# izhengfan/se2lam

Measured on AMD Instinct MI355X. Metric: BA GN-iters/s (200 KF, 20k pts), higher is better.
Workload: dtype f64; 1 GPU; globalBA-window 200 KF / 20000 landmarks / 119817 EdgeSE2XYZ + 199 PreEdgeSE2, LM optimize(10) (config 4 formulation, SURVEY D3); parallelism=single GPU

## Files before the change

### include/se2gpu.h

```cpp
#ifndef SE2GPU_H
#define SE2GPU_H

#include <stddef.h>
#include <stdint.h>

#ifdef __cplusplus
extern "C" {
#endif

#define SE2GPU_OK 0
#define SE2GPU_ERR_INVALID (-1)
#define SE2GPU_ERR_NO_DEVICE (-2)
#define SE2GPU_ERR_HIP (-3)
#define SE2GPU_ERR_CAPACITY (-4)
#define SE2GPU_ERR_STATE (-5)

const char* se2gpu_last_error(void);
int se2gpu_device_count(void);
const char* se2gpu_version(void);

typedef struct se2gpu_orb se2gpu_orb;

typedef struct se2gpu_orb_params {
    int32_t nfeatures;
// ... 255 lines not shown
#define SE2GPU_BA_GN 1
int se2gpu_ba_optimize(se2gpu_ba* h, int iters, int mode, const volatile uint8_t* stop_flag, int verbose,
                       se2gpu_ba_stats* stats);
int se2gpu_ba_optimize_batch(se2gpu_ba** handles, int count, int iters, int mode, const volatile uint8_t* stop_flag,
                             se2gpu_ba_stats* stats);
int se2gpu_ba_last_batch_path(void);
int se2gpu_ba_get_se2(se2gpu_ba* h, int id, double xyt[3]);
int se2gpu_ba_get_xyz(se2gpu_ba* h, int id, double xyz[3]);
int se2gpu_ba_get_all(se2gpu_ba* h, double* poses , double* lms );
double se2gpu_ba_chi2(se2gpu_ba* h);

int se2gpu_ba_debug_reduced_system(se2gpu_ba* h, double lambda, double* S, double* bs);
int se2gpu_ba_debug_solve(se2gpu_ba* h, double lambda, double* x, int* factor_ok);
int se2gpu_ba_debug_solver_path(const se2gpu_ba* h);
int se2gpu_ba_debug_linearize_counts(const se2gpu_ba* h, int* runs, int* skips, long long* twin_bytes);
int se2gpu_ba_debug_pool_sizes(int out2[2]);
int se2gpu_ba_debug_chol_verify(se2gpu_ba* h, unsigned long long* counts2, unsigned long long* records, int cap);
int se2gpu_ba_debug_solve_plan(int P, int D, const uint8_t* pattern, int allow_nd, int* nsys, int* nbc, int* depth, int* ntask,
                               int* ndep, int32_t* pose_off, int32_t* tasks4, int task_cap, int32_t* deps, int dep_cap);
int se2gpu_ba_debug_solve_plan_tile(int P, int D, const uint8_t* pattern, int allow_nd, int tile, int* nsys, int* nbc, int* depth, int* ntask,
                                    int* ndep, int32_t* pose_off, int32_t* tasks4, int task_cap, int32_t* deps, int dep_cap);
int se2gpu_ba_debug_solve_plan_neager(int P, int D, const uint8_t* pattern, int allow_nd, int tile, int32_t* neager, int cap);
int se2gpu_ba_debug_plan_neager(se2gpu_ba* h, int* nsys, int* permuted, int* ntask, int32_t* neager, int cap);

int se2gpu_triangulate(int n, const se2gpu_keypoint* kps_ref, const se2gpu_keypoint* kps_cur, int n_cur,
                       int32_t* match_idx, const uint8_t* has_observation, const float* P_ref, const float* P_cur,
                       const float* Ocam, float lower_depth, float upper_depth, int min_degree, float* pos_out,
                       uint8_t* good_parallax, int* n_good, int* n_tracked_old);

typedef struct se2gpu_track se2gpu_track;
int se2gpu_track_create(se2gpu_track** out);
void se2gpu_track_destroy(se2gpu_track* h);
int se2gpu_track_fundamental_mask(se2gpu_track* h, const float* pt1, const float* pt2, int n, uint8_t* mask,
                                  int* n_inliers);
int se2gpu_track_remove_outliers(se2gpu_track* h, const se2gpu_keypoint* kps1, int n1, const se2gpu_keypoint* kps2,
                                 int n2, int32_t* matches, int* n_inliers);
int se2gpu_track_last_ransac(const se2gpu_track* h, int info[4]);
int se2gpu_track_set_stream(se2gpu_track* h, void* hip_stream);
void* se2gpu_track_stream(se2gpu_track* h);
int se2gpu_track_sync(se2gpu_track* h);

int se2gpu_track_loop_verify_batch_device(se2gpu_track* h,
                                          const se2gpu_keypoint* d_kps, const int32_t* d_counts, int cap, int nframes,
                                          const uint8_t* d_has_mp ,
                                          const int32_t* d_num_mps ,
                                          const int32_t* d_pair_a, const int32_t* d_pair_b, int npairs,
// ... 123 lines not shown
```

### se2lam_amd/capi.py

```python
from __future__ import annotations

import ctypes as C
import os

import numpy as np

HERE = os.path.dirname(os.path.abspath(__file__))
LIB_PATH = os.path.join(HERE, "lib", "libse2gpu.so")

OK = 0
ERR_INVALID, ERR_NO_DEVICE, ERR_HIP, ERR_CAPACITY, ERR_STATE = -1, -2, -3, -4, -5


class Se2GpuError(RuntimeError):
    def __init__(self, code, msg):
        super().__init__(f"se2gpu error {code}: {msg}")
        self.code = code


class Keypoint(C.Structure):
    _fields_ = [("x", C.c_float), ("y", C.c_float), ("size", C.c_float), ("angle", C.c_float),
                ("response", C.c_float), ("octave", C.c_int32), ("class_id", C.c_int32)]


# ... 151 lines not shown
    "se2gpu_feat_edge_batch": (_I, [_I, _I, _I, _I, _VP, _VP, _D, _D, _D, _VP, _VP, _VP, _VP, _D, _D, _VP, _VP, _VP, _VP, _VP,
                                    _VP, _VP, _VP]),
    "se2gpu_ba_initialize": (_I, [_VP]),
    "se2gpu_ba_set_edge_level": (_I, [_VP, _I, _I]),
    "se2gpu_ba_reset_estimates": (_I, [_VP]),
    "se2gpu_ba_reset_estimates_batch": (_I, [_VP, _I]),
    "se2gpu_ba_optimize": (_I, [_VP, _I, _I, _PU8, _I, C.POINTER(BaStats)]),
    "se2gpu_ba_optimize_batch": (_I, [C.POINTER(_VP), _I, _I, _I, _PU8, C.POINTER(BaStats)]),
    "se2gpu_ba_last_batch_path": (_I, []),
    "se2gpu_ba_get_se2": (_I, [_VP, _I, _PD]),
    "se2gpu_ba_get_xyz": (_I, [_VP, _I, _PD]),
    "se2gpu_ba_get_all": (_I, [_VP, _PD, _PD]),
    "se2gpu_ba_chi2": (_D, [_VP]),
    "se2gpu_ba_debug_reduced_system": (_I, [_VP, _D, _PD, _PD]),
    "se2gpu_ba_debug_solve": (_I, [_VP, _D, _PD, C.POINTER(C.c_int)]),
    "se2gpu_ba_debug_solver_path": (_I, [_VP]),
    "se2gpu_ba_debug_linearize_counts": (_I, [_VP, C.POINTER(C.c_int), C.POINTER(C.c_int), C.POINTER(C.c_longlong)]),
    "se2gpu_ba_debug_chol_verify": (_I, [_VP, _VP, _VP, _I]),
    "se2gpu_ba_debug_pool_sizes": (_I, [_VP]),
    "se2gpu_ba_debug_solve_plan": (_I, [_I, _I, _VP, _I, _VP, _VP, _VP, _VP, _VP, _VP, _VP, _I, _VP, _I]),
    "se2gpu_ba_debug_solve_plan_tile": (_I, [_I, _I, _VP, _I, _I, _VP, _VP, _VP, _VP, _VP, _VP, _VP, _I, _VP, _I]),
    "se2gpu_ba_debug_solve_plan_neager": (_I, [_I, _I, _VP, _I, _I, _VP, _I]),
    "se2gpu_ba_debug_plan_neager": (_I, [_VP, C.POINTER(C.c_int), C.POINTER(C.c_int), C.POINTER(C.c_int), _VP, _I]),
    "se2gpu_triangulate": (_I, [_I, _VP, _VP, _I, _VP, _VP, _VP, _VP, _VP, C.c_float, C.c_float, _I, _VP, _VP,
                           C.POINTER(C.c_int), C.POINTER(C.c_int)]),
    "se2gpu_track_create": (_I, [C.POINTER(_VP)]),
    "se2gpu_track_destroy": (None, [_VP]),
    "se2gpu_track_fundamental_mask": (_I, [_VP, _VP, _VP, _I, _VP, C.POINTER(C.c_int)]),
    "se2gpu_track_remove_outliers": (_I, [_VP, _VP, _I, _VP, _I, _VP, C.POINTER(C.c_int)]),
    "se2gpu_track_last_ransac": (_I, [_VP, _VP]),
    "se2gpu_track_set_stream": (_I, [_VP, _VP]),
    "se2gpu_track_stream": (_VP, [_VP]),
    "se2gpu_track_sync": (_I, [_VP]),
    "se2gpu_track_loop_verify_batch_device": (_I, [_VP, _VP, _VP, _I, _I, _VP, _VP, _VP, _VP, _I, _VP, _VP, _VP, _VP]),
    "se2gpu_plane_motion_prior": (_I, [_VP, _VP, _D, _D, _D, _VP, _VP]),
    "se2gpu_track_pose_ba": (_I, [_VP, _VP, _VP, _VP, _I, _VP, _VP, _VP, _D, _D, _D, _D, _I, _VP, C.POINTER(BaStats)]),
    "se2gpu_track_triangulate": (_I, [_VP, _I, _VP, _VP, _I, _VP, _VP, _VP, _VP, _VP, C.c_float, C.c_float, _I, _VP, _VP,
                                 C.POINTER(C.c_int), C.POINTER(C.c_int)]),
    "se2gpu_ba_reduce_buffer_doubles": (_SZ, [_VP, _I]),
    "se2gpu_ba_exchange_doubles": (_SZ, [_I]),
    "se2gpu_ba_exchange_doubles_h": (_SZ, [_VP]),
    "se2gpu_ba_exchange_row": (_I, [_I, C.POINTER(C.c_size_t), C.POINTER(C.c_int)]),
    "se2gpu_ba_set_allreduce": (_I, [_VP, ALLREDUCE_FN, _VP, _VP]),
    "se2gpu_ba_set_shard": (_I, [_VP, _I, _I]),
    "se2gpu_comm_unique_id": (_I, [_VP]),
    "se2gpu_comm_create": (_I, [_VP, _I, _I, C.POINTER(_VP)]),
# ... 208 lines not shown
```

### se2lam_amd/csrc/ba.hip

```cpp
#include <algorithm>
#include <atomic>
#include <chrono>
#include <cmath>
#include <cstdlib>
#include <functional>
#include <limits>
#include <mutex>
#include <thread>
#include <memory>
#include <unordered_map>

#include "common.h"
#include "se3_math.h"
#include "ba_device.h"
#include "ba3_device.h"
#include "ba_window.h"

using namespace se2gpu;
using namespace se2gpu::badev;

namespace {



// ... 591 lines not shown
    }
}

constexpr int kGrpPerWG = 28;
constexpr int kChunk = 16;

struct Reduce2Args {
    int P, ld, nwg_off;
    double lambda;
    int root;
    const int4* grp;
    const int *blk_a, *blk_b, *pair_i, *pair_j, *blk_odo;
    const double *W, *Dg;
    const uint8_t* fixed;
    const int *pose_ptr, *pose_edges, *podo_ptr, *podo_item, *o_i, *o_j;
    const double *o_meas, *o_info, *poses;
    double *S, *bp;
    const BaCtl* ctl;
    const double* poses_b;
    unsigned* epoch;
    const int* pose_off;
    int nsys;
    const double *W_alt, *Dg_alt;
};
__device__ __forceinline__ void d_reduce2(const unsigned bx, const Reduce2Args& ra) {
    const double *W = ra.W, *Dg = ra.Dg, *poses = ra.poses;
    if (ra.ctl && ra.ctl->rec_sel) { W = ra.W_alt; Dg = ra.Dg_alt; }
    double lambda = ra.lambda;
    const int n = ra.pose_off ? ra.nsys : 3 * ra.P;
    __shared__ double part[kGrpPerWG][9];
    __shared__ double dpart[kBlock / 64][12];
    const int ndiag = (ra.P + 1 + 7) & ~7;
    if ((int)bx >= ndiag) {
        const int bid = (int)bx - ndiag;
        const int nwg_pad = (ra.nwg_off + 7) & ~7;
        const int wg = (bid & 7) * (nwg_pad >> 3) + (bid >> 3);
        if (wg >= ra.nwg_off) return;
        const int lane = threadIdx.x & 63, gw = lane / 9, en = lane - 9 * gw;
        const int g = gw < 7 ? (int)(threadIdx.x >> 6) * 7 + gw : kGrpPerWG;
        int4 d = make_int4(-1, 0, 0, 0);
        if (g < kGrpPerWG) d = ra.grp[(size_t)wg * kGrpPerWG + g];
        if (ra.ctl) {
            if (ra.ctl->done) return;
            if (ra.ctl->sel) poses = ra.poses_b;
        }
        const int r = en / 3, c = en - 3 * r;
        double acc0 = 0, acc1 = 0;
        int a = 0, b = 0, od = -1, ca = 0, cb = 0;
        bool free_ab = false;
        if (d.x >= 0) {
            const int gb = 9 * gw, t8 = min(en, 7);
            int q0 = min(d.y + t8, d.z - 1), q1 = min(d.y + 8 + t8, d.z - 1);
            int my_i0 = 0, my_j0 = 0, my_i1 = 0, my_j1 = 0;
            if (d.z > d.y) { my_i0 = ra.pair_i[q0]; my_j0 = ra.pair_j[q0]; my_i1 = ra.pair_i[q1]; my_j1 = ra.pair_j[q1]; }
            a = ra.blk_a[d.x];
            b = ra.blk_b[d.x];
            od = ra.blk_odo[d.x];
            free_ab = !ra.fixed[a] && !ra.fixed[b];
            ca = ra.pose_off ? ra.pose_off[a] : 3 * a;
            cb = ra.pose_off ? ra.pose_off[b] : 3 * b;
            for (int q = d.y; q < d.z; q += 8) {
                const bool second = ((q - d.y) & 8) != 0;
                if (!second && q != d.y) {
                    q0 = min(q + t8, d.z - 1); q1 = min(q + 8 + t8, d.z - 1);
                    my_i0 = ra.pair_i[q0]; my_j0 = ra.pair_j[q0]; my_i1 = ra.pair_i[q1]; my_j1 = ra.pair_j[q1];
                }
                const int my_i = second ? my_i1 : my_i0, my_j = second ? my_j1 : my_j0;
                double wi[8], wj[8];
#pragma unroll
                for (int u = 0; u < 8; ++u) {
                    const int ia = __shfl(my_i, gb + u), ib = __shfl(my_j, gb + u);
                    wi[u] = W[(size_t)ia * 9 + en];
                    wj[u] = W[(size_t)ib * 9 + en];
                }
#pragma unroll
                for (int u = 0; u < 8; u += 2) {
                    const double w0 = (q + u < d.z) ? 1.0 : 0.0, w1 = (q + u + 1 < d.z) ? 1.0 : 0.0;
                    double y[2][3], hh[2][3];
#pragma unroll
                    for (int k = 0; k < 3; ++k) {
                        y[0][k] = __shfl(wi[u], gb + 3 * r + k);
                        hh[0][k] = __shfl(wj[u], gb + 3 * c + k);
                        y[1][k] = __shfl(wi[u + 1], gb + 3 * r + k);
                        hh[1][k] = __shfl(wj[u + 1], gb + 3 * c + k);
                    }
                    acc0 += w0 * (y[0][0] * hh[0][0] + y[0][1] * hh[0][1] + y[0][2] * hh[0][2]);
                    acc1 += w1 * (y[1][0] * hh[1][0] + y[1][1] * hh[1][1] + y[1][2] * hh[1][2]);
                }
            }
            part[g][en] = acc0 + acc1;
        }
        __syncthreads();
        if (d.x >= 0 && (d.w & 0xff) == g) {
            const int ng = d.w >> 8;
            double tot = 0;
            for (int t = 0; t < ng; ++t) tot += part[g + t][en];
            double out = 0.0;
            if (free_ab) {
                out = -tot;
                if (od >= 0) {
                    double e[3], A[9], B[9], WA[9], WB[9], omr[3];
                    odo_terms(poses, ra.fixed, ra.o_i, ra.o_j, ra.o_meas, ra.o_info, od >> 1, e, A, B, WA, WB, omr);
                    const int rr = (od & 1) ? c : r, cc = (od & 1) ? r : c;
                    const double a0 = rr == 0 ? A[0] : (rr == 1 ? A[1] : A[2]), a1 = rr == 0 ? A[3] : (rr == 1 ? A[4] : A[5]),
                                 a2 = rr == 0 ? A[6] : (rr == 1 ? A[7] : A[8]);
                    const double b0 = cc == 0 ? WB[0] : (cc == 1 ? WB[1] : WB[2]), b1 = cc == 0 ? WB[3] : (cc == 1 ? WB[4] : WB[5]),
                                 b2 = cc == 0 ? WB[6] : (cc == 1 ? WB[7] : WB[8]);
                    out += a0 * b0 + a1 * b1 + a2 * b2;
                }
            }
            ra.S[(size_t)(ca + r) * ra.ld + cb + c] = out;
            ra.S[(size_t)(cb + c) * ra.ld + ca + r] = out;
        }
        return;
    }
    if (ra.ctl) {
        if (ra.ctl->done) return;
        if (ra.ctl->sel) poses = ra.poses_b;
        lambda = ra.ctl->lambda;
    }
    const int p = (int)bx;
    if (p > ra.P) return;
    const int lane = threadIdx.x & 63, wv = threadIdx.x >> 6;
    double* __restrict__ bs = ra.S + (size_t)n * ra.ld;
    if (p == ra.P) {
        for (size_t t = (size_t)n * ra.ld + n + threadIdx.x; t < (size_t)ra.ld * ra.ld; t += kBlock) ra.S[t] = 0.0;
        if (threadIdx.x == 0) {
            ra.S[(size_t)ra.ld * ra.ld + 2] = 0.0;
            *ra.epoch += 1u;
        }
        return;
// ... 66 lines not shown
            for (int q = 0; q < 3; ++q) {
                const double j0 = isj ? B[3 * q] : A[3 * q], j1 = isj ? B[3 * q + 1] : A[3 * q + 1], j2 = isj ? B[3 * q + 2] : A[3 * q + 2];
                const double w0 = isj ? WB[3 * q] : WA[3 * q], w1 = isj ? WB[3 * q + 1] : WA[3 * q + 1], w2 = isj ? WB[3 * q + 2] : WA[3 * q + 2];
                jr[q] = r == 0 ? j0 : (r == 1 ? j1 : j2);
                wc[q] = i < 9 ? (c == 0 ? w0 : (c == 1 ? w1 : w2)) : omr[q];
            }
            v += jr[0] * wc[0] + jr[1] * wc[1] + jr[2] * wc[2];
        }
        if (i < 9) {
            const int r = i / 3, c = i - 3 * r;
            double out;
            if (fa) out = (r == c && ra.root) ? 1.0 : 0.0;
            else out = v + ((r == c && ra.root) ? lambda : 0.0);
            const int cp = ra.pose_off ? ra.pose_off[p] : 3 * p;
            ra.S[(size_t)(cp + r) * ra.ld + cp + c] = out;
        } else {
            const int r = i - 9;
            const double gz = dpart[0][9 + r] + dpart[1][9 + r] + dpart[2][9 + r] + dpart[3][9 + r];
            bs[(ra.pose_off ? ra.pose_off[p] : 3 * p) + r] = fa ? 0.0 : v - gz;
            ra.bp[(size_t)p * 3 + r] = fa ? 0.0 : v;
        }
    }
}
__global__ __launch_bounds__(kBlock) void k_reduce2(Reduce2Args a) {
    d_reduce2(blockIdx.x, a);
}

__global__ void k_reduce_odo(int O, int ld, const int* __restrict__ o_i, const int* __restrict__ o_j,
                             const double* __restrict__ Oij, double* __restrict__ S, const int* __restrict__ pose_off) {
    const int t = blockIdx.x * blockDim.x + threadIdx.x;
    if (t >= O * 9) return;
    const int k = t / 9, r = (t % 9) / 3, c = t % 3;
    const int i = o_i[k], j = o_j[k];
    const double v = Oij[t];
    if (v == 0.0) return;
    const int ci = pose_off ? pose_off[i] : 3 * i, cj = pose_off ? pose_off[j] : 3 * j;
    atomicAdd(&S[(size_t)(ci + r) * ld + cj + c], v);
    atomicAdd(&S[(size_t)(cj + c) * ld + ci + r], v);
}

constexpr int kNB = 32;
constexpr int kSlabs = 4;
constexpr int kSlabDoubles = 2 * kNB * 8;
__host__ __device__ inline size_t pub_tile(int kind, int i, int j, int nt, int nbc) {
    return ((size_t)(kind * nt + i) * nbc + j) * (kSlabs * kSlabDoubles);
}
inline size_t chol_work_doubles(int ld) {
// ... 1847 lines not shown
    int bulk_E = 0;
    const int32_t *bulk_kf = nullptr, *bulk_lm = nullptr;
    const double *bulk_uv = nullptr, *bulk_info = nullptr;
    bool lg_active = false;
    std::vector<float> lg_lc, lg_lw, lg_sigma2, lg_Rcw, lg_twb;
    float lg_fx = 0, lg_srot = 0, lg_sz = 0;
    DevBuf<float> d_lg_lc, d_lg_lw, d_lg_sigma2, d_lg_Rcw, d_lg_twb;
    std::vector<EdgeOdo> odo;
    bool initialized = false;
    unsigned long init_serial = 0;
    hipEvent_t join_event = nullptr;
    hipStream_t join_stream = nullptr;
    bool own_pending = false;
    int P = 0, L = 0, E = 0, O = 0, nblk = 0, nparts = 0;
    int ld = 0;
    bool host_solve = false;
    DevBuf<double> poses0, lms0, poses_a, poses_b, lms_a, lms_b;
    double *poses = nullptr, *poses_t = nullptr, *lms = nullptr, *lms_t = nullptr;
    DevBuf<uint8_t> fixed;
    DevBuf<int> lm_ptr, e_kf, e_lm, pose_ptr, pose_edges, podo_ptr, podo_item, o_i, o_j;
    DevBuf<int> blk_a, blk_b, blk_ptr, pair_i, pair_j, blk_odo;
    DevBuf<int4> grp;
    int nwg_off = 0, grp_cap_wg = 0;
    DevBuf<uint8_t> garena;
    DevBuf<int> plan_np, plan_base, plan_key0, plan_key1, plan_idx, plan_hist, plan_offs, plan_out, plan_tsum, plan_toff;
    DevBuf<int2> plan_st0, plan_st1;
    bool odo_fallback = false;
    bool odo_self_loop = false;
    DevBuf<double> e_uv, e_info, o_meas, o_info;
    DevBuf<double> Hpl, Hpp_e, bp_e, Hll, bl, Dinv, z, Y, Dg, Hpp, bp, Oii, Ojj, Oij, obi, obj;
    DevBuf<double> red_own, xp, part, scal, diag3, Rinv;
    DevBuf<double> rec_twin;
    bool run_spec = false;
    DevBuf<double> red_packed;
    DevBuf<int4> chol_tasks;
    DevBuf<int> chol_deps;
    DevBuf<int> chol_neager;
    DevBuf<int> pose_off;
    DevBuf<int> col_src;
    std::vector<int> h_pose_off;
    DevBuf<uint8_t> plan_nz;
    DevBuf<double> plan_nzd;
    PinBuf<uint8_t> h_plan_nz;
    DevBuf<uint8_t> solver_arena;
    int nsys = 0;
    int solve_depth = 0;
// ... 740 lines not shown
        const int w = w_cyc;
        for (int lv = 0; lv <= 2; ++lv) ring(w, w, lv);
        auto tiles = [&](int poses) { return (D * poses + nb - 1) / nb; };
        int sw_best = w, est_best = tiles(std::max(h - w, P - h - w)) + tiles(2 * w);
        for (int sw = w + 1; sw <= w + nb && 2 * sw + 2 * min_interior <= P; ++sw) {
            const int est = tiles(std::max(h - sw, P - h - sw)) + tiles(2 * sw);
            if (est < est_best) { est_best = est; sw_best = sw; }
        }
        if (sw_best != w) ring(w, sw_best, 0);
    }
}

int ba_copy_stream(int device, hipStream_t* out) {
    static std::mutex mu;
    static hipStream_t streams[64] = {};
    std::lock_guard<std::mutex> lk(mu);
    SE2_REQUIRE(device >= 0 && device < 64, SE2GPU_ERR_INVALID, "device %d", device);
    if (!streams[device]) SE2_HIP(hipStreamCreateWithFlags(&streams[device], hipStreamNonBlocking));
    *out = streams[device];
    return SE2GPU_OK;
}

int ba_allreduce(se2gpu_ba* h, double* ptr, size_t count);

int ba_upload_graph(se2gpu_ba* h) {
    static const bool trace = env_flag("SE2GPU_BA_INIT_TRACE", false);
    const auto t_begin = std::chrono::steady_clock::now();
    auto lap = [&](const char* what) {
        if (trace)
            std::fprintf(stderr, "[ba init] %-28s %8.1f us\n", what,
                         std::chrono::duration<double, std::micro>(std::chrono::steady_clock::now() - t_begin).count());
    };
    const int P = (int)h->pose_ids.size(), L = (int)h->lm_ids.size();
    const int E = h->bulk_E ? h->bulk_E : (int)h->he_kf.size(), O_in = h->model ? (int)h->odo3.size() : (int)h->odo.size();
    const int D = h->D, ps = h->ps, gpw = h->model ? kGrpPerWG3 : kGrpPerWG;
    const int DS = D * (D + 1) / 2;
    SE2_REQUIRE(P > 0, SE2GPU_ERR_STATE, "initialize: no pose vertices");
    SE2_REQUIRE(!h->model || (h->world == 1 && !h->allreduce), SE2GPU_ERR_STATE, "the SE3 model is single-GPU");
    SE2_REQUIRE(h->have_cam, SE2GPU_ERR_STATE, "initialize: add_cam was not called");
    SE2_REQUIRE(!h->huber_mixed, SE2GPU_ERR_INVALID, "all EdgeSE2XYZ must share one Huber delta (Map.cpp:977)");
    h->P = P; h->L = L; h->E = E; h->O = O_in;
    h->cam.huber = E ? h->huber_delta : 0.0;
    h->cam3 = Cam3{h->cam.fx, h->cam.cx, h->cam.cy, h->cam.huber};
    for (int i = 0; i < 3; ++i)
        for (int j = 0; j < 3; ++j) h->cam.Rcb[i * 3 + j] = h->Rbc[j * 3 + i];
    for (int i = 0; i < 3; ++i)
// ... 478 lines not shown
        static const bool verify = env_flag("SE2GPU_BA_CHOL_VERIFY", false);
        if (verify) {
            const size_t words = kVfyChk + 2 * 2 * kSlabs * (size_t)nt2 * nbc2;
            SE2_CHECK(h->chol_vfy.reserve(words));
            SE2_HIP(hipMemsetAsync(h->chol_vfy.p, 0, words * sizeof(unsigned long long), st));
        } else {
            h->chol_vfy.release();
        }
        h->chol_steps = env_is("SE2GPU_BA_CHOL", "steps") || nt2 > 64 || h->chol_fallback;
        if (env_flag("SE2GPU_BA_CHOL_TRACE", false)) {
            SE2_CHECK(h->chol_trace.reserve(16 * (size_t)h->chol_ntask));
            SE2_HIP(hipMemsetAsync(h->chol_trace.p, 0, 16 * (size_t)h->chol_ntask * sizeof(long long), st));
        }
        lap("solve plan");
    }
    SE2_HIP(hipStreamSynchronize(st));
    if (device_plan) {
        int nwg = 0;
        std::memcpy(&nwg, h->h_scal.p, sizeof(int));
        SE2_REQUIRE(nwg <= h->grp_cap_wg, SE2GPU_ERR_CAPACITY, "device plan: %d workgroups exceed the bound %d", nwg, h->grp_cap_wg);
        h->nwg_off = std::max(nwg, 1);
    }
    lap("synchronise");
    h->bulk_E = 0;
    h->bulk_kf = h->bulk_lm = nullptr;
    h->bulk_uv = h->bulk_info = nullptr;
    h->initialized = true;
    h->est_valid = false;
    static std::atomic<unsigned long> serial{0};
    h->init_serial = ++serial;
    drain.armed = false;
    return SE2GPU_OK;
}


int ba_join(se2gpu_ba* h, hipStream_t st, hipEvent_t* ev) {
    if (h->join_event) {
        if (h->join_stream != st) SE2_HIP(hipStreamWaitEvent(st, h->join_event, 0));
        h->join_event = nullptr;
        h->join_stream = nullptr;
    }
    if (h->own_pending && h->stream != st) {
        if (!*ev) SE2_HIP(hipEventCreateWithFlags(ev, hipEventDisableTiming));
        SE2_HIP(hipEventRecord(*ev, h->stream));
        SE2_HIP(hipStreamWaitEvent(st, *ev, 0));
        h->own_pending = false;
// ... 57 lines not shown
inline double* ba_scal(se2gpu_ba* h) { return h->red + (size_t)h->ld * h->ld; }
inline dim3 upd_grid(const se2gpu_ba* h) { return grid1((size_t)h->L * kGroup, kBlock); }
inline dim3 reduce2_grid(const se2gpu_ba* h) { return dim3(((h->P + 1 + 7) & ~7) + ((h->nwg_off + 7) & ~7)); }
LinArgs lin_args(se2gpu_ba* h, const Bufs& B, double lambda, const RecSet& alt) {
    return LinArgs{h->cam, h->L, h->lm_ptr.p, h->e_kf.p, h->e_uv.p, h->e_info.p, B.pa, h->fixed.p, B.la, h->Hpl.p, h->Hpp_e.p,
                   h->bp_e.p, h->Hll.p, h->bl.p, lambda, h->Dinv.p, h->z.p, h->Dg.p, B.c, B.pb, B.lb, alt};
}
OdoArgs odo_args(se2gpu_ba* h, const double* poses, bool ctl) {
    const Bufs B = bufs(h, ctl);
    return OdoArgs{h->O, h->o_i.p, h->o_j.p, h->o_meas.p, h->o_info.p, ctl ? B.pa : poses, h->fixed.p, h->Oii.p, h->Ojj.p, h->Oij.p,
                   h->obi.p, h->obj.p, B.c, ctl ? B.pb : nullptr};
}
PoseReduceArgs pose_reduce_args(se2gpu_ba* h) {
    return PoseReduceArgs{h->P, h->pose_ptr.p, h->pose_edges.p, h->Hpp_e.p, h->bp_e.p, h->podo_ptr.p, h->podo_item.p, h->Oii.p,
                          h->Ojj.p, h->obi.p, h->obj.p, h->Hpp.p, h->bp.p};
}
MaxdiagArgs maxdiag_args(se2gpu_ba* h, int dpp, int stride9, BaCtl* ctl) {
    return MaxdiagArgs{h->L, h->Hll.p, h->P, stride9 ? h->Hpp.p : h->diag3.p, h->fixed.p, h->scal.p, dpp, stride9, ctl};
}
Reduce2Args reduce2_args(se2gpu_ba* h, const Bufs& B, double lambda, const RecSet& alt) {
    return Reduce2Args{h->P, h->ld, h->nwg_off, lambda, h->root, h->grp.p, h->blk_a.p, h->blk_b.p, h->pair_i.p, h->pair_j.p,
                       h->blk_odo.p, h->Hpl.p, h->Dg.p, h->fixed.p, h->pose_ptr.p, h->pose_edges.p, h->podo_ptr.p, h->podo_item.p,
                       h->o_i.p, h->o_j.p, h->o_meas.p, h->o_info.p, B.pa, h->red, h->bp.p, B.c, B.pb, &h->ctl.p->epoch,
                       h->pose_off.p, h->nsys, alt.W, alt.Dg};
}
CholArgs chol_args(se2gpu_ba* h, const BaCtl* ctl, int skip, unsigned long long* head, bool verify) {
    const int n = h->nsys, ld = h->ld;
    const int nt = ld / kNB, nbc = (n + kNB - 1) / kNB;
    double* YU = h->Rinv.p + 2 * (size_t)nt * nbc * kSlabs * kSlabDoubles;
    unsigned* flagA = h->chol_flags.p;
    return CholArgs{h->red, h->Rinv.p, YU, ld, n, nbc, h->chol_tasks.p + skip, h->chol_deps.p, h->chol_neager.p + skip, h->col_src.p,
                    flagA, flagA + kSlabs * (size_t)nt * nbc, &h->ctl.p->epoch, ba_scal(h) + 2, h->chol_trace.p, ctl, h->xp.p,
                    verify ? h->chol_vfy.p : nullptr, head, h->chol_ntask - skip};
}
TrialEnd trial_end(se2gpu_ba* h, const Bufs& B, int step, int decide, int notify, double seq, bool lin = false, bool post = true) {
    return TrialEnd{ba_scal(h), post ? h->d_mail : nullptr, seq, B.c ? h->ctl.p : nullptr,
                    B.c ? (const volatile int*)h->d_stop : nullptr, step, decide, notify, lin ? 1 : 0};
}
FinArgs fin_args(se2gpu_ba* h, const Bufs& B, const double* xp, const TrialEnd& te) {
    return FinArgs{1, (int)upd_grid(h).x, h->P, h->O, h->root, h->fixed.p, xp, h->bp.p, B.pa, B.pb,
                   h->o_i.p, h->o_j.p, h->o_meas.p, h->o_info.p, h->fin_counter.p, te};
}
UpdArgs upd_args(se2gpu_ba* h, const Bufs& B, double lambda, const double* xp, const FinArgs& fin, bool lin = false) {
    return UpdArgs{h->cam, h->L, lambda, h->lm_ptr.p, h->e_kf.p, h->e_uv.p, h->e_info.p, B.pa, h->fixed.p, B.la, xp, h->z.p, h->Hpl.p,
                   h->bl.p, B.lb, h->part.p, B.c, B.pb, fin, h->Dinv.p,
                   lin ? SpecArgs{{rec_own(h), rec_twin(h)}, h->Hpp_e.p, h->bp_e.p} : SpecArgs{}};
}
// ... 1228 lines not shown
                               int* ndep, int32_t* pose_off, int32_t* tasks4, int task_cap, int32_t* deps, int dep_cap) {
    SE2_REQUIRE(P > 0 && (D == 3 || D == 6) && nsys && nbc && depth && ntask && ndep, SE2GPU_ERR_INVALID, "debug_solve_plan: bad argument");
    SolvePlan sp;
    solve_plan_choose(P, D, pattern, allow_nd != 0, sp);
    *nsys = sp.nsys; *nbc = sp.nbc; *depth = sp.depth; *ntask = (int)sp.tasks.size(); *ndep = (int)sp.deps.size();
    if (pose_off) std::memcpy(pose_off, sp.pose_off.data(), (size_t)P * 4);
    if (tasks4) {
        SE2_REQUIRE(task_cap >= (int)sp.tasks.size(), SE2GPU_ERR_CAPACITY, "debug_solve_plan: %zu tasks", sp.tasks.size());
        std::memcpy(tasks4, sp.tasks.data(), sp.tasks.size() * sizeof(int4));
    }
    if (deps) {
        SE2_REQUIRE(dep_cap >= (int)sp.deps.size(), SE2GPU_ERR_CAPACITY, "debug_solve_plan: %zu dependency entries", sp.deps.size());
        std::memcpy(deps, sp.deps.data(), sp.deps.size() * 4);
    }
    return SE2GPU_OK;
}

int se2gpu_ba_debug_solve_plan_neager(int P, int D, const uint8_t* pattern, int allow_nd, int tile, int32_t* neager, int cap) {
    SE2_REQUIRE(P > 0 && (D == 3 || D == 6) && (tile == 32 || tile == 64) && neager, SE2GPU_ERR_INVALID, "debug_solve_plan_neager: bad argument");
    SolvePlan sp;
    solve_plan_choose(P, D, pattern, allow_nd != 0, sp, false, tile);
    SE2_REQUIRE(cap >= (int)sp.neager.size(), SE2GPU_ERR_CAPACITY, "debug_solve_plan_neager: %zu tasks", sp.neager.size());
    std::memcpy(neager, sp.neager.data(), sp.neager.size() * 4);
    return SE2GPU_OK;
}

int se2gpu_ba_debug_plan_neager(se2gpu_ba* h, int* nsys, int* permuted, int* ntask, int32_t* neager, int cap) {
    SE2_REQUIRE(h && h->initialized && nsys && permuted && ntask, SE2GPU_ERR_STATE, "debug_plan_neager before initialize");
    SE2_CHECK(ba_join(h));
    SE2_HIP(hipStreamSynchronize(h->stream));
    *nsys = h->nsys; *permuted = h->col_src.p ? 1 : 0; *ntask = h->chol_ntask;
    if (neager) {
        SE2_REQUIRE(cap >= h->chol_ntask && h->chol_neager.p, SE2GPU_ERR_CAPACITY, "debug_plan_neager: %d tasks", h->chol_ntask);
        SE2_HIP(hipMemcpy(neager, h->chol_neager.p, (size_t)h->chol_ntask * 4, hipMemcpyDeviceToHost));
    }
    return SE2GPU_OK;
}

int se2gpu_ba_debug_chol_verify(se2gpu_ba* h, unsigned long long* counts2, unsigned long long* records, int cap) {
    SE2_REQUIRE(h && h->initialized && h->chol_vfy.p, SE2GPU_ERR_STATE, "the handle does not verify its hand-offs (SE2GPU_BA_CHOL_VERIFY=1)");
    SE2_CHECK(ba_join(h));
    SE2_HIP(hipStreamSynchronize(h->stream));
    unsigned long long head[8];
    SE2_HIP(hipMemcpy(head, h->chol_vfy.p, sizeof(head), hipMemcpyDeviceToHost));
    counts2[0] = head[0]; counts2[1] = head[1];
    const int nrec = (int)std::min<unsigned long long>(std::min<unsigned long long>(head[0], kVfyRecords), (unsigned long long)std::max(cap, 0));
// ... 673 lines not shown
```

Measured before the change: 7346 iters/s.

## Precompute flat per-group index records for reduce2 off-diagonal blocks

At graph upload a new kernel builds, for each reduce group, a flat 11-int4 record holding block offsets, the odometry index, the fixed flag and the pair indices, so the off-diagonal reduce path replaces chains of dependent gathers with a few contiguous loads. The odometry block term is now computed before the landmark loop and stored in shared memory, so its latency overlaps the main accumulation. The kernel also gets a min-occupancy launch bound of 5. The trade-off is extra device memory and a small setup kernel, plus possible register pressure from the occupancy hint. It is enabled by default through an environment flag.

```diff
diff --git a/include/se2gpu.h b/include/se2gpu.h
--- a/include/se2gpu.h
+++ b/include/se2gpu.h
@@ -301,6 +301,10 @@
                                     int* ndep, int32_t* pose_off, int32_t* tasks4, int task_cap, int32_t* deps, int dep_cap);
 int se2gpu_ba_debug_solve_plan_neager(int P, int D, const uint8_t* pattern, int allow_nd, int tile, int32_t* neager, int cap);
 int se2gpu_ba_debug_plan_neager(se2gpu_ba* h, int* nsys, int* permuted, int* ntask, int32_t* neager, int cap);
+int se2gpu_ba_debug_flat_records_host(int nslots, const int32_t* grp4, const int32_t* blk_a, const int32_t* blk_b, const int32_t* blk_odo,
+                                      const int32_t* pair_i, const int32_t* pair_j, const uint8_t* fixed, const int32_t* pose_off,
+                                      const int32_t* o_i, const int32_t* o_j, int32_t* flat);
+int se2gpu_ba_debug_flat_records(se2gpu_ba* h, int32_t* grp4, int32_t* flat, int cap_slots, int* nslots);
 
 int se2gpu_triangulate(int n, const se2gpu_keypoint* kps_ref, const se2gpu_keypoint* kps_cur, int n_cur,
                        int32_t* match_idx, const uint8_t* has_observation, const float* P_ref, const float* P_cur,
diff --git a/profiles/ba_reduce_flat/stamp_patch.py b/profiles/ba_reduce_flat/stamp_patch.py
--- /dev/null
+++ b/profiles/ba_reduce_flat/stamp_patch.py
@@ -0,0 +1,48 @@
+import sys
+src, dst = sys.argv[1], sys.argv[2]
+s = open(src).read()
+
+def rep(old, new, count=1):
+    global s
+    assert s.count(old) >= 1, old
+    s = s.replace(old, new, count)
+
+rep("constexpr int kFlatQ = 11;",
+    """constexpr int kFlatQ = 11;
+__device__ long long g_r2_stamps[4096 * 8];
+#define R2S(i) do { if (threadIdx.x == 0 && bx < 4096) g_r2_stamps[(size_t)bx * 8 + (i)] = wall_clock64(); } while (0)
+#define R2S_T(i, T) do { if ((int)threadIdx.x == (T) && bx < 4096) g_r2_stamps[(size_t)bx * 8 + (i)] = wall_clock64(); } while (0)
+#define R2USE(v) asm volatile("" ::"v"(v))""")
+rep("        const int wg = (bid & 7) * (nwg_pad >> 3) + (bid >> 3);\n        if (wg >= ra.nwg_off) return;",
+    "        const int wg = (bid & 7) * (nwg_pad >> 3) + (bid >> 3);\n        if (wg >= ra.nwg_off) return;\n        R2S(0);")
+rep("        const int r = en / 3, c = en - 3 * r;\n        double acc0 = 0, acc1 = 0;",
+    "        R2USE(d.x); R2USE(fq.x);\n        R2S(1);\n        const int r = en / 3, c = en - 3 * r;\n        double acc0 = 0, acc1 = 0;")
+rep("            // The block's PreEdgeSE2 term (the group that combines the block adds it): with the flat record",
+    "            R2USE(my_i0); R2USE(my_j1); R2USE(ca); R2USE(cb); R2USE(od);\n            R2S(2);\n            // The block's PreEdgeSE2 term (the group that combines the block adds it): with the flat record")
+rep("            // The group loads every word ONCE", "            R2S(3);\n            // The group loads every word ONCE")
+rep("                    acc1 += w1 * (y[1][0] * hh[1][0] + y[1][1] * hh[1][1] + y[1][2] * hh[1][2]);\n                }\n            }\n            part[g][en] = acc0 + acc1;",
+    "                    acc1 += w1 * (y[1][0] * hh[1][0] + y[1][1] * hh[1][1] + y[1][2] * hh[1][2]);\n                }\n                if (q == d.y) { R2USE(acc0); R2USE(acc1); R2S(4); }\n            }\n            R2USE(acc0); R2USE(acc1);\n            R2S(5);\n            part[g][en] = acc0 + acc1;")
+rep("        __syncthreads();\n        if (d.x >= 0 && (d.w & 0xff) == g) {\n            const int ng = d.w >> 8;",
+    "        __syncthreads();\n        R2S(6);\n        if (d.x >= 0 && (d.w & 0xff) == g) {\n            const int ng = d.w >> 8;")
+rep("            ra.S[(size_t)(cb + c) * ra.ld + ca + r] = out;\n        }\n        return;",
+    "            ra.S[(size_t)(cb + c) * ra.ld + ca + r] = out;\n            R2USE(out);\n        }\n        R2S(7);\n        return;")
+rep("    double acc[12] = {0, 0, 0, 0, 0, 0, 0, 0, 0, 0, 0, 0};  // S diag (6 sym), bp (3), g (3)",
+    "    R2S(0);\n    double acc[12] = {0, 0, 0, 0, 0, 0, 0, 0, 0, 0, 0, 0};  // S diag (6 sym), bp (3), g (3)")
+rep("            o[9 + r] = J[r] * omr[0] + J[3 + r] * omr[1] + J[6 + r] * omr[2];\n        }\n    }",
+    "            o[9 + r] = J[r] * omr[0] + J[3 + r] * omr[1] + J[6 + r] * omr[2];\n        }\n        R2S_T(3, kBlock - 8);\n    }")
+rep("                ee[u] = ra.pose_edges[e0 + min(t, ne - 1)];\n            }",
+    "                ee[u] = ra.pose_edges[e0 + min(t, ne - 1)];\n            }\n            if (base == 0) { R2USE(ee[0]); R2USE(ee[3]); R2S(1); }")
+rep("#pragma unroll\n    for (int i = 0; i < 12; ++i) acc[i] = wave_sum(acc[i]);",
+    "    R2USE(acc[0]); R2USE(acc[11]);\n    R2S(2);\n#pragma unroll\n    for (int i = 0; i < 12; ++i) acc[i] = wave_sum(acc[i]);")
+rep("    __syncthreads();\n    if (threadIdx.x < 12) {  // entries 0..8",
+    "    __syncthreads();\n    R2S(6);\n    if (threadIdx.x < 12) {  // entries 0..8")
+rep("            ra.bp[(size_t)p * 3 + r] = fa ? 0.0 : v;\n        }\n    }\n}",
+    "            ra.bp[(size_t)p * 3 + r] = fa ? 0.0 : v;\n        }\n    }\n    R2S(7);\n}")
+rep("// k_plan_flat's record builder (flat_record, the function the kernel calls) on host arrays",
+    """extern "C" int se2gpu_ba_debug_reduce_stamps(long long* out, int n) {
+    SE2_HIP(hipDeviceSynchronize());
+    SE2_HIP(hipMemcpyFromSymbol(out, HIP_SYMBOL(g_r2_stamps), (size_t)n * sizeof(long long)));
+    return SE2GPU_OK;
+}
+// k_plan_flat's record builder (flat_record, the function the kernel calls) on host arrays""")
+open(dst, "w").write(s)
diff --git a/profiles/ba_reduce_flat/stamps_summary.py b/profiles/ba_reduce_flat/stamps_summary.py
--- /dev/null
+++ b/profiles/ba_reduce_flat/stamps_summary.py
@@ -0,0 +1,33 @@
+import numpy as np, sys
+for name in ("legacy","flat"):
+    z=np.load(f"{sys.argv[1]}/stamps_{name}.npz")
+    S=z["stamps"]; P=int(z["P"]); ndiag=(P+1+7)&~7
+    print("==",name,"runs",S.shape[0],"flat_slots",int(z["flat_slots"]))
+    for run in range(S.shape[0]):
+        st=S[run].astype(np.int64)
+        valid=(st[:,0]>0)&(st[:,7]>0)
+        t0=st[valid,0].min()
+        rel=(st-t0)*0.01
+        diag=np.zeros(4096,bool); diag[:P]=True; diag&=valid
+        off=np.zeros(4096,bool); off[ndiag:]=True; off&=valid
+        end=rel[valid,7].max()
+        print(f"run {run}: valid {valid.sum()} diag {diag.sum()} off {off.sum()}  kernel span (first start -> last end) {end:.2f} us; last end: diag {rel[diag,7].max():.2f} off {rel[off,7].max():.2f}; starts: diag max {rel[diag,0].max():.2f} off max {rel[off,0].max():.2f}")
+        o=rel[off]
+        seg=[("start->record/grp",0,1),("->indices/blk",1,2),("->(odo before loop)",2,3),("->W round 1",3,4),("->all rounds",4,5),("->barrier",5,6),("->end(odo+store)",6,7)]
+        def q(x): return "med %.2f p90 %.2f max %.2f"%(np.median(x),np.percentile(x,90),x.max())
+        for nm,a,b in seg:
+            ok=(o[:,a]>-1e5)&(o[:,b]>-1e5)&(st[off][:,a]>0)&(st[off][:,b]>0)
+            print("   off %-22s %s  (n=%d)"%(nm,q(o[ok,b]-o[ok,a]),ok.sum()))
+        print("   off total                 ",q(o[:,7]-o[:,0]))
+        idx=np.argsort(o[:,7])[-max(10,len(o)//20):]
+        print("   off LAST 5%% to end: start med %.2f; tail seg (barrier->end) med %.2f max %.2f; total med %.2f"%(np.median(o[idx,0]),np.median(o[idx,7]-o[idx,6]),(o[idx,7]-o[idx,6]).max(),np.median(o[idx,7]-o[idx,0])))
+        long_tail=(o[:,7]-o[:,6])>0.8
+        print("   off wgs with barrier->end > 0.8us: %d, their end med %.2f max %.2f ; others end med %.2f max %.2f"%(long_tail.sum(), np.median(o[long_tail,7]) if long_tail.any() else -1, o[long_tail,7].max() if long_tail.any() else -1, np.median(o[~long_tail,7]), o[~long_tail,7].max()))
+        dg=rel[diag]; sd=st[diag]
+        ok1=(sd[:,1]>0)&(sd[:,2]>0)
+        print("   diag start->idx %s (n=%d)"%(q(dg[ok1,1]-dg[ok1,0]),ok1.sum()))
+        print("   diag idx->Dg gathered %s (n=%d)"%(q(dg[ok1,2]-dg[ok1,1]),ok1.sum()))
+        ok=sd[:,3]>0
+        print("   diag start->odo lanes done %s (n=%d)"%(q(dg[ok,3]-dg[ok,0]),ok.sum()))
+        print("   diag start->gather done %s"%q(dg[:,2]-dg[:,0]))
+        print("   diag gather->barrier %s ; barrier->end %s ; total %s"%(q(dg[:,6]-dg[:,2]),q(dg[:,7]-dg[:,6]),q(dg[:,7]-dg[:,0])))
diff --git a/se2lam_amd/capi.py b/se2lam_amd/capi.py
--- a/se2lam_amd/capi.py
+++ b/se2lam_amd/capi.py
@@ -197,6 +197,8 @@
     "se2gpu_ba_debug_solve_plan_tile": (_I, [_I, _I, _VP, _I, _I, _VP, _VP, _VP, _VP, _VP, _VP, _VP, _I, _VP, _I]),
     "se2gpu_ba_debug_solve_plan_neager": (_I, [_I, _I, _VP, _I, _I, _VP, _I]),
     "se2gpu_ba_debug_plan_neager": (_I, [_VP, C.POINTER(C.c_int), C.POINTER(C.c_int), C.POINTER(C.c_int), _VP, _I]),
+    "se2gpu_ba_debug_flat_records_host": (_I, [_I, _VP, _VP, _VP, _VP, _VP, _VP, _VP, _VP, _VP, _VP, _VP]),
+    "se2gpu_ba_debug_flat_records": (_I, [_VP, _VP, _VP, _I, C.POINTER(C.c_int)]),
     "se2gpu_triangulate": (_I, [_I, _VP, _VP, _I, _VP, _VP, _VP, _VP, _VP, C.c_float, C.c_float, _I, _VP, _VP,
                            C.POINTER(C.c_int), C.POINTER(C.c_int)]),
     "se2gpu_track_create": (_I, [C.POINTER(_VP)]),
diff --git a/se2lam_amd/csrc/ba.hip b/se2lam_amd/csrc/ba.hip
--- a/se2lam_amd/csrc/ba.hip
+++ b/se2lam_amd/csrc/ba.hip
@@ -637,13 +637,61 @@
     const int* pose_off;
     int nsys;
     const double *W_alt, *Dg_alt;
+    const int4* flat;
 };
+constexpr int kFlatQ = 11;
+__host__ __device__ inline void flat_record(const int4 d, const int* blk_a, const int* blk_b, const int* blk_odo,
+                                            const int* pair_i, const int* pair_j, const uint8_t* fixed, const int* pose_off,
+                                            const int* o_i, const int* o_j, int4* rec) {
+    rec[0] = d;
+    for (int t = 1; t < kFlatQ; ++t) rec[t] = make_int4(0, 0, 0, 0);
+    rec[1].z = -1;
+    if (d.x < 0) return;
+    const int a = blk_a[d.x], b = blk_b[d.x], od = blk_odo[d.x];
+    rec[1] = make_int4(pose_off ? pose_off[a] : 3 * a, pose_off ? pose_off[b] : 3 * b, od, (!fixed[a] && !fixed[b]) ? 1 : 0);
+    if (od >= 0) rec[2] = make_int4(o_i[od >> 1], o_j[od >> 1], 0, 0);
+    if (d.z > d.y)
+        for (int t = 0; t < 8; ++t) {
+            const int last = d.z - 1, q0 = d.y + t < last ? d.y + t : last, q1 = d.y + 8 + t < last ? d.y + 8 + t : last;
+            rec[3 + t] = make_int4(pair_i[q0], pair_j[q0], pair_i[q1], pair_j[q1]);
+        }
+}
+struct PlanFlatArgs {
+    int ngrp;
+    const int4* grp;
+    const int *blk_a, *blk_b, *blk_odo, *pair_i, *pair_j;
+    const uint8_t* fixed;
+    const int *pose_off, *o_i, *o_j;
+    int4* flat;
+};
+__global__ __launch_bounds__(256) void k_plan_flat(PlanFlatArgs a) {
+    const int t = blockIdx.x * 256 + threadIdx.x;
+    if (t < a.ngrp)
+        flat_record(a.grp[t], a.blk_a, a.blk_b, a.blk_odo, a.pair_i, a.pair_j, a.fixed, a.pose_off, a.o_i, a.o_j,
+                    a.flat + (size_t)t * kFlatQ);
+}
+__device__ __forceinline__ __attribute__((flatten)) void odo_terms_regs(const double pij[6], const double meas[3], const double* info, double e[3],
+                                               double A[9], double B[9], double WA[9], double WB[9], double omr[3]) {
+    const int zero = 0, one = 1;
+    odo_terms(pij, nullptr, &zero, &one, meas, info, 0, e, A, B, WA, WB, omr);
+}
+__device__ __forceinline__ double odo_block_entry(const double pij[6], const double meas[3], const double* info, int od, int r, int c) {
+    double e[3], A[9], B[9], WA[9], WB[9], omr[3];
+    odo_terms_regs(pij, meas, info, e, A, B, WA, WB, omr);
+    const int rr = (od & 1) ? c : r, cc = (od & 1) ? r : c;
+    const double a0 = rr == 0 ? A[0] : (rr == 1 ? A[1] : A[2]), a1 = rr == 0 ? A[3] : (rr == 1 ? A[4] : A[5]),
+                 a2 = rr == 0 ? A[6] : (rr == 1 ? A[7] : A[8]);
+    const double b0 = cc == 0 ? WB[0] : (cc == 1 ? WB[1] : WB[2]), b1 = cc == 0 ? WB[3] : (cc == 1 ? WB[4] : WB[5]),
+                 b2 = cc == 0 ? WB[6] : (cc == 1 ? WB[7] : WB[8]);
+    return a0 * b0 + a1 * b1 + a2 * b2;
+}
 __device__ __forceinline__ void d_reduce2(const unsigned bx, const Reduce2Args& ra) {
     const double *W = ra.W, *Dg = ra.Dg, *poses = ra.poses;
     if (ra.ctl && ra.ctl->rec_sel) { W = ra.W_alt; Dg = ra.Dg_alt; }
     double lambda = ra.lambda;
     const int n = ra.pose_off ? ra.nsys : 3 * ra.P;
     __shared__ double part[kGrpPerWG][9];
+    __shared__ double odo_part[kGrpPerWG][9];
     __shared__ double dpart[kBlock / 64][12];
     const int ndiag = (ra.P + 1 + 7) & ~7;
     if ((int)bx >= ndiag) {
@@ -653,8 +701,15 @@
         if (wg >= ra.nwg_off) return;
         const int lane = threadIdx.x & 63, gw = lane / 9, en = lane - 9 * gw;
         const int g = gw < 7 ? (int)(threadIdx.x >> 6) * 7 + gw : kGrpPerWG;
-        int4 d = make_int4(-1, 0, 0, 0);
-        if (g < kGrpPerWG) d = ra.grp[(size_t)wg * kGrpPerWG + g];
+        int4 d = make_int4(-1, 0, 0, 0), fb = make_int4(0, 0, -1, 0), fo = make_int4(0, 0, 0, 0), fq = make_int4(0, 0, 0, 0);
+        if (g < kGrpPerWG) {
+            if (ra.flat) {
+                const int4* rec = ra.flat + ((size_t)wg * kGrpPerWG + g) * kFlatQ;
+                d = rec[0]; fb = rec[1]; fo = rec[2]; fq = rec[3 + min(en, 7)];
+            } else {
+                d = ra.grp[(size_t)wg * kGrpPerWG + g];
+            }
+        }
         if (ra.ctl) {
             if (ra.ctl->done) return;
             if (ra.ctl->sel) poses = ra.poses_b;
@@ -665,15 +720,31 @@
         bool free_ab = false;
         if (d.x >= 0) {
             const int gb = 9 * gw, t8 = min(en, 7);
-            int q0 = min(d.y + t8, d.z - 1), q1 = min(d.y + 8 + t8, d.z - 1);
-            int my_i0 = 0, my_j0 = 0, my_i1 = 0, my_j1 = 0;
-            if (d.z > d.y) { my_i0 = ra.pair_i[q0]; my_j0 = ra.pair_j[q0]; my_i1 = ra.pair_i[q1]; my_j1 = ra.pair_j[q1]; }
-            a = ra.blk_a[d.x];
-            b = ra.blk_b[d.x];
-            od = ra.blk_odo[d.x];
-            free_ab = !ra.fixed[a] && !ra.fixed[b];
-            ca = ra.pose_off ? ra.pose_off[a] : 3 * a;
-            cb = ra.pose_off ? ra.pose_off[b] : 3 * b;
+            int q0, q1, my_i0 = 0, my_j0 = 0, my_i1 = 0, my_j1 = 0;
+            if (ra.flat) {
+                my_i0 = fq.x; my_j0 = fq.y; my_i1 = fq.z; my_j1 = fq.w;
+                ca = fb.x; cb = fb.y; od = fb.z;
+                free_ab = fb.w != 0;
+            } else {
+                q0 = min(d.y + t8, d.z - 1); q1 = min(d.y + 8 + t8, d.z - 1);
+                if (d.z > d.y) { my_i0 = ra.pair_i[q0]; my_j0 = ra.pair_j[q0]; my_i1 = ra.pair_i[q1]; my_j1 = ra.pair_j[q1]; }
+                a = ra.blk_a[d.x];
+                b = ra.blk_b[d.x];
+                od = ra.blk_odo[d.x];
+                free_ab = !ra.fixed[a] && !ra.fixed[b];
+                ca = ra.pose_off ? ra.pose_off[a] : 3 * a;
+                cb = ra.pose_off ? ra.pose_off[b] : 3 * b;
+            }
+            if (ra.flat && free_ab && od >= 0 && (d.w & 0xff) == g) {
+                double opij[6], omeas[3];
+#pragma unroll
+                for (int t = 0; t < 3; ++t) {
+                    opij[t] = poses[3 * (size_t)fo.x + t];
+                    opij[3 + t] = poses[3 * (size_t)fo.y + t];
+                    omeas[t] = ra.o_meas[3 * (size_t)(od >> 1) + t];
+                }
+                odo_part[g][en] = odo_block_entry(opij, omeas, ra.o_info + 9 * (size_t)(od >> 1), od, r, c);
+            }
             for (int q = d.y; q < d.z; q += 8) {
                 const bool second = ((q - d.y) & 8) != 0;
                 if (!second && q != d.y) {
@@ -714,14 +785,18 @@
             if (free_ab) {
                 out = -tot;
                 if (od >= 0) {
-                    double e[3], A[9], B[9], WA[9], WB[9], omr[3];
-                    odo_terms(poses, ra.fixed, ra.o_i, ra.o_j, ra.o_meas, ra.o_info, od >> 1, e, A, B, WA, WB, omr);
-                    const int rr = (od & 1) ? c : r, cc = (od & 1) ? r : c;
-                    const double a0 = rr == 0 ? A[0] : (rr == 1 ? A[1] : A[2]), a1 = rr == 0 ? A[3] : (rr == 1 ? A[4] : A[5]),
-                                 a2 = rr == 0 ? A[6] : (rr == 1 ? A[7] : A[8]);
-                    const double b0 = cc == 0 ? WB[0] : (cc == 1 ? WB[1] : WB[2]), b1 = cc == 0 ? WB[3] : (cc == 1 ? WB[4] : WB[5]),
-                                 b2 = cc == 0 ? WB[6] : (cc == 1 ? WB[7] : WB[8]);
-                    out += a0 * b0 + a1 * b1 + a2 * b2;
+                    if (ra.flat) {
+                        out += odo_part[g][en];
+                    } else {
+                        double e[3], A[9], B[9], WA[9], WB[9], omr[3];
+                        odo_terms(poses, ra.fixed, ra.o_i, ra.o_j, ra.o_meas, ra.o_info, od >> 1, e, A, B, WA, WB, omr);
+                        const int rr = (od & 1) ? c : r, cc = (od & 1) ? r : c;
+                        const double a0 = rr == 0 ? A[0] : (rr == 1 ? A[1] : A[2]), a1 = rr == 0 ? A[3] : (rr == 1 ? A[4] : A[5]),
+                                     a2 = rr == 0 ? A[6] : (rr == 1 ? A[7] : A[8]);
+                        const double b0 = cc == 0 ? WB[0] : (cc == 1 ? WB[1] : WB[2]), b1 = cc == 0 ? WB[3] : (cc == 1 ? WB[4] : WB[5]),
+                                     b2 = cc == 0 ? WB[6] : (cc == 1 ? WB[7] : WB[8]);
+                        out += a0 * b0 + a1 * b1 + a2 * b2;
+                    }
                 }
             }
             ra.S[(size_t)(ca + r) * ra.ld + cb + c] = out;
@@ -834,7 +909,7 @@
         }
     }
 }
-__global__ __launch_bounds__(kBlock) void k_reduce2(Reduce2Args a) {
+__global__ __launch_bounds__(kBlock, 5) void k_reduce2(Reduce2Args a) {
     d_reduce2(blockIdx.x, a);
 }
 
@@ -2728,6 +2803,9 @@
     DevBuf<int> blk_a, blk_b, blk_ptr, pair_i, pair_j, blk_odo;
     DevBuf<int4> grp;
     int nwg_off = 0, grp_cap_wg = 0;
+    DevBuf<int4> grp_flat;
+    size_t flat_slots = 0;
+    bool flat_on = false;
     DevBuf<uint8_t> garena;
     DevBuf<int> plan_np, plan_base, plan_key0, plan_key1, plan_idx, plan_hist, plan_offs, plan_out, plan_tsum, plan_toff;
     DevBuf<int2> plan_st0, plan_st1;
@@ -3514,6 +3592,7 @@
 }
 
 int ba_allreduce(se2gpu_ba* h, double* ptr, size_t count);
+bool ba_env_reduce_flat() { return env_flag("SE2GPU_BA_REDUCE_FLAT", true); }
 
 int ba_upload_graph(se2gpu_ba* h) {
     static const bool trace = env_flag("SE2GPU_BA_INIT_TRACE", false);
@@ -4038,6 +4117,18 @@
         h->nwg_off = std::max(nwg, 1);
     }
     lap("synchronise");
+    h->flat_on = h->model == 0 && ba_env_reduce_flat();
+    if (h->flat_on) {
+        const size_t slots = (size_t)h->nwg_off * gpw;
+        SE2_CHECK(h->grp_flat.reserve(slots * kFlatQ));
+        h->flat_slots = slots;
+        const PlanFlatArgs fa{(int)slots, h->grp.p, h->blk_a.p, h->blk_b.p, h->blk_odo.p, h->pair_i.p, h->pair_j.p,
+                              h->fixed.p, h->pose_off.p, h->o_i.p, h->o_j.p, h->grp_flat.p};
+        hipLaunchKernelGGL(k_plan_flat, grid1(slots, 256), dim3(256), 0, st, fa);
+        SE2_HIP(hipGetLastError());
+        SE2_HIP(hipStreamSynchronize(st));
+        lap("flat records");
+    }
     h->bulk_E = 0;
     h->bulk_kf = h->bulk_lm = nullptr;
     h->bulk_uv = h->bulk_info = nullptr;
@@ -4141,7 +4232,7 @@
     return Reduce2Args{h->P, h->ld, h->nwg_off, lambda, h->root, h->grp.p, h->blk_a.p, h->blk_b.p, h->pair_i.p, h->pair_j.p,
                        h->blk_odo.p, h->Hpl.p, h->Dg.p, h->fixed.p, h->pose_ptr.p, h->pose_edges.p, h->podo_ptr.p, h->podo_item.p,
                        h->o_i.p, h->o_j.p, h->o_meas.p, h->o_info.p, B.pa, h->red, h->bp.p, B.c, B.pb, &h->ctl.p->epoch,
-                       h->pose_off.p, h->nsys, alt.W, alt.Dg};
+                       h->pose_off.p, h->nsys, alt.W, alt.Dg, h->flat_on ? h->grp_flat.p : nullptr};
 }
 CholArgs chol_args(se2gpu_ba* h, const BaCtl* ctl, int skip, unsigned long long* head, bool verify) {
     const int n = h->nsys, ld = h->ld;
@@ -5416,6 +5507,30 @@
     solve_plan_choose(P, D, pattern, allow_nd != 0, sp, false, tile);
     SE2_REQUIRE(cap >= (int)sp.neager.size(), SE2GPU_ERR_CAPACITY, "debug_solve_plan_neager: %zu tasks", sp.neager.size());
     std::memcpy(neager, sp.neager.data(), sp.neager.size() * 4);
+    return SE2GPU_OK;
+}
+
+int se2gpu_ba_debug_flat_records_host(int nslots, const int32_t* grp4, const int32_t* blk_a, const int32_t* blk_b, const int32_t* blk_odo,
+                                      const int32_t* pair_i, const int32_t* pair_j, const uint8_t* fixed, const int32_t* pose_off,
+                                      const int32_t* o_i, const int32_t* o_j, int32_t* flat) {
+    SE2_REQUIRE(nslots >= 0 && grp4 && blk_a && blk_b && blk_odo && fixed && flat, SE2GPU_ERR_INVALID, "debug_flat_records_host: bad argument");
+    for (int s = 0; s < nslots; ++s) {
+        int4 rec[kFlatQ];
+        flat_record(make_int4(grp4[4 * s], grp4[4 * s + 1], grp4[4 * s + 2], grp4[4 * s + 3]), blk_a, blk_b, blk_odo, pair_i, pair_j,
+                    fixed, pose_off, o_i, o_j, rec);
+        std::memcpy(flat + (size_t)s * 4 * kFlatQ, rec, sizeof(rec));
+    }
+    return SE2GPU_OK;
+}
+int se2gpu_ba_debug_flat_records(se2gpu_ba* h, int32_t* grp4, int32_t* flat, int cap_slots, int* nslots) {
+    SE2_REQUIRE(h && h->initialized && nslots, SE2GPU_ERR_STATE, "debug_flat_records before initialize");
+    *nslots = h->flat_on ? (int)h->flat_slots : 0;
+    if (!grp4 || !flat || !h->flat_on) return SE2GPU_OK;
+    SE2_REQUIRE(cap_slots >= *nslots, SE2GPU_ERR_CAPACITY, "debug_flat_records: %d slots", *nslots);
+    SE2_CHECK(ba_join(h));
+    SE2_HIP(hipStreamSynchronize(h->stream));
+    SE2_HIP(hipMemcpy(grp4, h->grp.p, h->flat_slots * sizeof(int4), hipMemcpyDeviceToHost));
+    SE2_HIP(hipMemcpy(flat, h->grp_flat.p, h->flat_slots * kFlatQ * sizeof(int4), hipMemcpyDeviceToHost));
     return SE2GPU_OK;
 }
 
```

After: 7434 iters/s (median of 6 runs). 1.01x the previous value.
